# sjpark0905/DNA-LDPC-codes

Hardware: NVIDIA B200
Metric: decoded Gbit/s, n=18432 prprp (higher is better)
Workload: dtype f64

## Files before the change

dna-ldpc-codes_b200/__init__.py:

```python
import ctypes as C
import os

import numpy as np

_HERE = os.path.dirname(os.path.abspath(__file__))
LIB_PATH = os.environ.get("DNALDPC_LIB") or os.path.join(_HERE, "libdnaldpc.so")

OK = 0
PREC_F64, PREC_F32 = 0, 1
IN_LR_F64, IN_LLR_F64, IN_BSC_BITS, IN_AWGN_F32, IN_AWGN_F64, IN_VOTE_I8 = range(6)
FLAG_HOST_EXP = 1
FLAG_FIXED_ITERS = 2
FLAG_MINSUM = 4
FLAG_LAYERED = 8

EXPORTS = [
    "dnaldpc_last_error", "dnaldpc_version", "dnaldpc_code_read_pchk", "dnaldpc_code_from_csr",
    "dnaldpc_code_write_pchk", "dnaldpc_code_free", "dnaldpc_code_dims", "dnaldpc_code_export",
    "dnaldpc_code_check_regular", "dnaldpc_decoder_create", "dnaldpc_decoder_destroy", "dnaldpc_decode_batch",
    "dnaldpc_decode_batch_device", "dnaldpc_run_bp_decoder", "dnaldpc_std_dev", "dnaldpc_vote_table",
    "dnaldpc_bsc_table", "dnaldpc_synth_bsc_device", "dnaldpc_get_stats", "dnaldpc_set_profiling",
    "dnaldpc_selftest_math", "dnaldpc_redecode_sweep", "dnaldpc_get_trace", "dnaldpc_decode_window",
    "dnaldpc_redecode_sweep_ex", "dnaldpc_synth_awgn_device", "dnaldpc_synth_vote_device", "dnaldpc_code_systematic",
    "dnaldpc_encode_device", "dnaldpc_encode", "dnaldpc_extract_device", "dnaldpc_extract", "dnaldpc_simulate",
# ... 7 lines not shown


class Input(C.Structure):
    _fields_ = [("kind", C.c_int32), ("flags", C.c_int32), ("data", C.c_void_p), ("frame_stride", C.c_size_t),
                ("param", C.c_double), ("table", C.c_void_p)]


class Output(C.Structure):
    _fields_ = [("bits", C.c_void_p), ("dblk", C.c_void_p), ("iters", C.c_void_p), ("is_codeword", C.c_void_p),
                ("posterior", C.c_void_p), ("pchk", C.c_void_p)]


class Stats(C.Structure):
    _fields_ = [("frames", C.c_int64), ("frame_iters", C.c_int64), ("kernel_launches", C.c_int64),
                ("waves", C.c_int64), ("row_ms", C.c_double), ("col_ms", C.c_double), ("total_ms", C.c_double),
                ("compactions", C.c_int64)]


class Window(C.Structure):
    _fields_ = [("code_type", C.c_int32), ("L", C.c_int32), ("w", C.c_int32), ("win", C.c_int32),
                ("Mv", C.c_void_p), ("Mc", C.c_void_p)]


class Sim(C.Structure):
    _fields_ = [("channel", C.c_int32), ("flags", C.c_int32), ("param", C.c_double), ("mean_reads", C.c_double),
                ("seed", C.c_uint64), ("max_iter", C.c_int32), ("max_frames", C.c_int64), ("target_frame_errors", C.c_int64)]


class SimResult(C.Structure):
    _fields_ = [(k, C.c_int64) for k in ("frames", "iterations", "frame_errors", "bit_errors", "msg_frame_errors",
                                         "msg_bit_errors", "detected", "undetected", "raw_frame_errors", "raw_bit_errors")]
# ... 350 lines not shown
```

dna-ldpc-codes_b200/csrc/bp_kernels.cuh:

```cuda
#pragma once
#include <cuda_runtime.h>
#include <stdint.h>

#include "bp_math.cuh"
#include "rng.cuh"

namespace dnaldpc {

constexpr int kFG = 32;

template <typename T> __device__ __forceinline__ T ld_stream(const T *p) { return __ldcs(p); }
template <typename T> __device__ __forceinline__ void st_stream(T *p, T v) { __stcs(p, v); }


template <typename T>
__device__ __noinline__ void row_slow_path(T *base, const T *lr_lane, const int32_t *cols, int deg, bool fresh) {
    auto pr_at = [&](int k) -> T { return fresh ? lr_lane[(size_t)cols[k] * kFG] : base[(size_t)k * kFG]; };
    T B = T(1);
    for (int k = deg - 1; k >= 0; k--) {
        T F = T(1);
        for (int m = 0; m < k; m++) F = mul_rn(F, check_factor_slow(pr_at(m)));
        const T dk = check_factor_slow(pr_at(k));
        base[(size_t)k * kFG] = check_to_bit_slow(mul_rn(F, B));
        B = mul_rn(B, dk);
// ... 323 lines not shown
    for (int i = 0; i < 8; i++) d[i] = __hiloint2double((int)w[2 * i + 1], (int)w[2 * i]);
    ck = __hiloint2double((int)w[17], (int)w[16]);
}

__device__ __forceinline__ int nth_set_bit8(uint32_t m, int r) {
    int f = 0;
#pragma unroll
    for (int q = 0; q < 8; q++) {
        if (q == r && m) f = __ffs(m) - 1;
        m &= m - 1;
    }
    return f;
}

constexpr int kTmWarps = 12;

template <int DC, int UR>
__global__ void __launch_bounds__(kTmWarps * 32, 1)
row_pass_tmem_kernel(double *__restrict__ msg, const double *__restrict__ lratio, const uint32_t *__restrict__ actw,
                     const uint32_t *__restrict__ freshw, const int32_t *__restrict__ col_idx, int M, int N, int E,
                     int g0, int G, unsigned int *__restrict__ job_counter, int l2_hint) {
    static_assert(DC % 8 == 0 && (DC / 8) * kTmBlockCols * (kTmWarps / 4) <= 512, "tensor-memory columns");
    constexpr uint32_t kTileBytes = DC * kFG * sizeof(double);
    constexpr int NB = DC / 8, NT = DC / 4, NI = (DC + 31) / 32;
    extern __shared__ __align__(128) unsigned char smem_raw[];
    const int lane = threadIdx.x & 31, warp = threadIdx.x >> 5;
    double *tile = reinterpret_cast<double *>(smem_raw) + (size_t)warp * DC * kFG;
    unsigned char *aux = smem_raw + (size_t)kTmWarps * DC * kFG * sizeof(double);
    uint64_t *bar = reinterpret_cast<uint64_t *>(aux) + warp;
    int *sidx = reinterpret_cast<int *>(aux + kTmWarps * sizeof(uint64_t)) + warp * DC;
    uint32_t *tm_slot = reinterpret_cast<uint32_t *>(aux + kTmWarps * sizeof(uint64_t) + (size_t)kTmWarps * DC * sizeof(int));
    const double *col = tile + lane;
    const uint64_t policy = l2_evict_first_policy();
    if (warp == 0) tmem_alloc_512(tm_slot);
    if (lane == 0) {
        mbar_init(bar, 1);
        mbar_fence_init();
    }
    asm volatile("tcgen05.fence::before_thread_sync;" ::: "memory");
    __syncthreads();
    asm volatile("tcgen05.fence::after_thread_sync;" ::: "memory");
    const uint32_t tm_base = *tm_slot;
    const uint32_t taddr = tm_base + ((uint32_t)((warp & 3) * 32) << 16) + (uint32_t)((warp >> 2) * NB * kTmBlockCols);
    const unsigned njobs = (unsigned)M * (unsigned)G;
    const int kq = lane >> 3, rk = lane & 7;
    uint32_t phase = 0;

    auto start_item = [&](int g, int e0, uint32_t act, uint32_t fw, double (&v)[NT]) {
        const uint32_t fresh_mask = fw & act;
        if ((act & ~fresh_mask) != 0 && lane == 0) {
            asm volatile("fence.proxy.async.shared::cta;" ::: "memory");
            mbar_expect_tx(bar, kTileBytes);
            if (l2_hint) tma_load_1d_hint(tile, msg + ((size_t)g * E + e0) * kFG, kTileBytes, bar, policy);
            else tma_load_1d(tile, msg + ((size_t)g * E + e0) * kFG, kTileBytes, bar);
        }
        if (fresh_mask != 0) {
            const bool mine = rk < __popc(fresh_mask);
            const int f = nth_set_bit8(fresh_mask, rk);
            const double *lr_base = lratio + (size_t)g * N * kFG;
#pragma unroll
            for (int t = 0; t < NT; t++) v[t] = mine ? lr_base[(size_t)sidx[t * 4 + kq] * kFG + f] : 0.0;
        }
    };
    auto claim_raw = [&]() -> unsigned {
        unsigned j = 0;
        if (lane == 0) j = atomicAdd(job_counter, 1u);
        return j;
    };

    unsigned job = __shfl_sync(0xffffffffu, claim_raw(), 0);
    unsigned job_n = __shfl_sync(0xffffffffu, claim_raw(), 0);
    int g = 0, e0 = 0;
    uint32_t act = 0, fw = 0;
    double v[NT];
    if (job < njobs) {
        g = g0 + (int)(job / (unsigned)M);
        e0 = (int)(job % (unsigned)M) * DC;
        for (int k = lane; k < DC; k += 32) sidx[k] = __ldg(col_idx + e0 + k);
        __syncwarp();
        act = actw[g]; fw = freshw[g];
        if (act != 0) start_item(g, e0, act, fw, v);
    }
    while (job < njobs) {
        const unsigned raw_nn = claim_raw();
        const bool valid_n = job_n < njobs;
        const int g_n = g0 + (int)(job_n / (unsigned)M), e0_n = (int)(job_n % (unsigned)M) * DC;
        uint32_t act_n = 0, fw_n = 0;
        int idx_n[NI];
#pragma unroll
        for (int q = 0; q < NI; q++) idx_n[q] = 0;
        if (valid_n) {
            act_n = actw[g_n]; fw_n = freshw[g_n];
#pragma unroll
            for (int q = 0; q < NI; q++)
                if (lane + 32 * q < DC) idx_n[q] = __ldg(col_idx + e0_n + lane + 32 * q);
        }
        const bool on = (act >> lane) & 1u, fresh = (fw >> lane) & 1u;
        double *base = msg + ((size_t)g * E + e0) * kFG + lane;
        const double *lr_lane = lratio + (size_t)g * N * kFG + lane;
        const int32_t *cols_cur = col_idx + e0;
        bool bad = false;
        if (act != 0) {
            const uint32_t fresh_mask = fw & act;
            if ((act & ~fresh_mask) != 0) {
                mbar_wait(bar, phase);
                phase ^= 1u;
            }
            if (fresh_mask != 0) {
                const int nf = __popc(fresh_mask);
                {
                    const bool mine = rk < nf;
                    const int f = nth_set_bit8(fresh_mask, rk);
#pragma unroll
                    for (int t = 0; t < NT; t++)
                        if (mine) tile[(t * 4 + kq) * kFG + f] = v[t];
                }
                for (int r0 = 8; r0 < nf; r0 += 8) {
                    const int r = r0 + rk;
                    const bool mine = r < nf;
                    const int f = mine ? (int)__fns(fresh_mask, 0, r + 1) : 0;
                    double w[NT];
#pragma unroll
// ... 10 lines not shown
                double d8[8];
                const double ckb = B;
#pragma unroll
                for (int kk = 7; kk >= 0; kk--) {
                    const double dk = check_factor(col[(b * 8 + kk) * kFG], bad);
                    d8[kk] = dk;
                    B = mul_rn(B, dk);
                }
                tmem_st_block(taddr + (uint32_t)(b * kTmBlockCols), d8, ckb);
            }
            asm volatile("tcgen05.wait::st.sync.aligned;" ::: "memory");
        }
        __syncwarp();
#pragma unroll
        for (int q = 0; q < NI; q++)
            if (lane + 32 * q < DC) sidx[lane + 32 * q] = idx_n[q];
        __syncwarp();
        if (valid_n && act_n != 0) start_item(g_n, e0_n, act_n, fw_n, v);
        if (on && bad) row_slow_path<double>(base, lr_lane, cols_cur, DC, fresh);
        if (act != 0) {
            double F = 1.0;
            const bool store = on && !bad;
#pragma unroll(UR)
            for (int b = 0; b < NB; b++) {
                double d8[8], Bv[8];
                tmem_ld_block(taddr + (uint32_t)(b * kTmBlockCols), d8, Bv[7]);
#pragma unroll
                for (int kk = 7; kk > 0; kk--) Bv[kk - 1] = mul_rn(Bv[kk], d8[kk]);
#pragma unroll
                for (int kk = 0; kk < 8; kk++) {
                    const double t = mul_rn(F, Bv[kk]);
                    const double lr = check_to_bit(t);
                    if (store) st_stream(base + (size_t)(b * 8 + kk) * kFG, lr);
                    F = mul_rn(F, d8[kk]);
                }
            }
        }
        job = job_n; g = g_n; e0 = e0_n; act = act_n; fw = fw_n;
        asm volatile("shfl.sync.idx.b32 %0, %1, 0, 31, 0xffffffff;" : "=r"(job_n) : "r"(raw_nn));
    }
    asm volatile("tcgen05.fence::before_thread_sync;" ::: "memory");
    __syncthreads();
    if (warp == 0) tmem_dealloc_512(tm_base);
}

constexpr int kColWarps = 8;

template <typename T, int DV>
struct ColIn {
    int eid[DV];
    T lr[DV];
    T P;
    int deg;
};

// ... 165 lines not shown
    }
}

constexpr int kSynThreads = 256;
constexpr int kSynSplit = 64;

struct SynArgs {
    int32_t *iters_out;
    uint8_t *ok_out;
    int M, N, g0, max_iter, consider_new, fixed_iters;
    unsigned int *counter;
    unsigned int *finished;
    unsigned int *counters_to_zero;
    int clear_fresh;
    unsigned int *row_jobs;
};

constexpr int kCounterWords = 4;

__device__ __forceinline__ uint32_t syn_head(const SchedArrays &s, const SynArgs &a, int g, uint32_t &act) {
    if (a.counters_to_zero && blockIdx.x == 0 && blockIdx.y == 0 && threadIdx.x == 0) {
        a.counters_to_zero[0] = 0; a.counters_to_zero[1] = 0; a.counters_to_zero[2] = 0; a.counters_to_zero[3] = 0xffffffffu;
    }
    if (a.row_jobs && blockIdx.x == 0 && blockIdx.y == 0 && threadIdx.x == 0) *a.row_jobs = 0;
    act = s.actw[g];
    const uint32_t consider = a.consider_new ? s.newfw[g] : act;
    if (consider == 0 && a.counter && blockIdx.x == 0 && threadIdx.x == 0) {
        const unsigned add = (unsigned)(__popc(act) + __popc(s.donew[g]));
        if (add) atomicAdd(a.counter, add);
    }
    return consider;
}

template <int THREADS>
__device__ __forceinline__ void syn_tail(const SchedArrays &s, const SynArgs &a, int g, uint32_t act, uint32_t consider, uint32_t acc) {
    acc = __reduce_or_sync(0xffffffffu, acc);
    __shared__ uint32_t s_or[THREADS / 32];
    __shared__ unsigned int s_ticket;
    if ((threadIdx.x & 31) == 0) s_or[threadIdx.x >> 5] = acc;
// ... 501 lines not shown
```

dna-ldpc-codes_b200/csrc/capi.cu:

```cuda
#include <cuda_runtime.h>

#include <cmath>
#include <cstring>
#include <memory>
#include <string>
#include <thread>
#include <vector>

#include "../../include/dnaldpc.h"
#include "../host/code.h"
#include "../host/layers.h"
#include "../host/systematic.h"
#include "encoder.h"
#include "engine.h"
#include "sim.h"
#include "sources.h"

using namespace dnaldpc;

struct dnaldpc_code {
    Code c;
};
struct dnaldpc_decoder {
    Code c;
// ... 286 lines not shown
        o2.pchk = out->pchk ? t_pchk.data() : nullptr;
        rc = dnaldpc_decode_batch(d, &in2, (int64_t)K, max_iter, &o2);
        if (rc) return rc;
        for (size_t k = 0; k < K; k++) {
            const size_t f = (size_t)failed[k];
            if (out->bits) memcpy(out->bits + f * wpf, &t_bits[k * wpf], wpf * 4);
            if (out->dblk) memcpy(out->dblk + f * N, &t_dblk[k * (size_t)N], (size_t)N);
            if (out->iters) out->iters[f] = t_it[k];
            if (out->posterior) memcpy(out->posterior + f * N, &t_post[k * (size_t)N], (size_t)N * 8);
            if (out->pchk) memcpy(out->pchk + f * M, &t_pchk[k * (size_t)M], (size_t)M);
            ok[f] = t_ok[k];
            if (rounds) rounds[f] = r;
        }
        total.frames += d->stats.frames; total.frame_iters += d->stats.frame_iters;
        total.kernel_launches += d->stats.kernel_launches; total.waves += d->stats.waves;
        total.compactions += d->stats.compactions;
    }
    if (out->is_codeword) memcpy(out->is_codeword, ok.data(), (size_t)F);
    d->stats = total;
    return DNALDPC_OK;
}

int dnaldpc_redecode_sweep_ex(dnaldpc_decoder *d, const dnaldpc_input *in, int64_t F, int max_iter, const double *params,
                              int n_params, const dnaldpc_output *out, int32_t *rounds) {
    DeviceRestore restore_device;
    if (!d || !in || !out || !params || n_params <= 0 || F < 0 || max_iter < 0) return set_err(DNALDPC_ERR_ARG, "bad argument");
    if (F > 0 && !in->data) return set_err(DNALDPC_ERR_ARG, "null input buffer");
    if (in->kind == DNALDPC_IN_LR_F64) return set_err(DNALDPC_ERR_ARG, "a sweep needs a parameter to vary: LR_F64 inputs have none");
    if (in->kind == DNALDPC_IN_VOTE_I8 && in->table) return set_err(DNALDPC_ERR_ARG, "a vote-count sweep builds its tables from params[]: table must be NULL");
    for (int r = 0; r < n_params; r++) {
        dnaldpc_input t = *in;
// ... 203 lines not shown
```

dna-ldpc-codes_b200/csrc/engine.cu:

```cuda
#include "engine.h"

#include <algorithm>
#include <cmath>
#include <cstdio>
#include <cstdlib>
#include <cstring>
#include <thread>

#include "../host/layers.h"
#include "bp_kernels.cuh"
#include "layered_kernels.cuh"
#include "sw_kernels.cuh"

namespace dnaldpc {

#define CK(call)                                      \
    do {                                              \
        cudaError_t e_ = (call);                      \
        if (e_ != cudaSuccess) return fail(e_, #call); \
    } while (0)

int Engine::fail(cudaError_t e, const char *what) {
    err_ = std::string("CUDA error: ") + cudaGetErrorString(e) + " in " + what;
    return DNALDPC_ERR_CUDA;
// ... 75 lines not shown
    if (own_stream_) cudaStreamDestroy(own_stream_);
    for (auto &s : io_stream_) if (s) cudaStreamDestroy(s);
}

int Engine::ensure_slots(int G, bool want_post) {
    if (G > cap_groups_) {
        void *ptrs[] = {d_msg_, d_lratio_, d_post_, d_decw_, d_masks_, d_arrive_, d_slot_, d_mv_};
        for (void *p : ptrs) if (p) cudaFree(p);
        d_msg_ = d_lratio_ = d_post_ = nullptr; d_decw_ = d_masks_ = nullptr; d_arrive_ = nullptr; d_slot_ = d_mv_ = nullptr;
        cap_groups_ = 0;
        const size_t msg_elems = std::max<size_t>((size_t)E_, (size_t)M_ * layer_w_);
        CK(cudaMalloc(&d_msg_, std::max<size_t>((size_t)G * msg_elems * kFG * esz_, 16)));
        CK(cudaMalloc(&d_lratio_, (size_t)G * N_ * kFG * esz_));
        CK(cudaMalloc((void **)&d_decw_, (size_t)G * N_ * sizeof(uint32_t)));
        CK(cudaMalloc((void **)&d_masks_, (size_t)G * 6 * sizeof(uint32_t)));
        CK(cudaMalloc((void **)&d_arrive_, (size_t)G * sizeof(unsigned)));
        CK(cudaMalloc((void **)&d_slot_, (size_t)G * kFG * 4 * sizeof(int32_t)));
        CK(cudaMalloc((void **)&d_mv_, ((size_t)G * kFG * 2 + 2) * sizeof(int32_t)));
        cap_groups_ = G;
    }
    if (want_post && !d_post_) CK(cudaMalloc(&d_post_, (size_t)cap_groups_ * N_ * kFG * esz_));
    return DNALDPC_OK;
}

int Engine::ensure_frame_scratch(int64_t F) {
    if (F > cap_frames_) {
        if (d_iters_) cudaFree(d_iters_);
        if (d_ok_) cudaFree(d_ok_);
        d_iters_ = nullptr; d_ok_ = nullptr; cap_frames_ = 0;
        CK(cudaMalloc((void **)&d_iters_, (size_t)F * sizeof(int32_t)));
        CK(cudaMalloc((void **)&d_ok_, (size_t)F));
// ... 4 lines not shown

void Engine::fill_sched(SchedArrays &s) const {
    const size_t G = (size_t)cap_groups_;
    s.actw = d_masks_; s.donew = d_masks_ + G; s.newfw = d_masks_ + 2 * G; s.freshw = d_masks_ + 3 * G;
    s.harvw = d_masks_ + 4 * G; s.unsatw = d_masks_ + 5 * G;
    s.arrive = d_arrive_;
    const size_t S = G * kFG;
    s.slot_frame = d_slot_; s.slot_iter = d_slot_ + S; s.harv_frame = d_slot_ + 2 * S; s.harv_iter = d_slot_ + 3 * S;
    s.next_frame = d_next_;
    s.avail = d_next_ + 1;
    s.iter_sum = d_next_ + 2;
    s.in_row = d_rows_;
    s.out_row = d_rows_ + cap_rows_;
}


template <typename T> int Engine::launch_row(int g0, int G, cudaStream_t st) {
    T *msg = (T *)d_msg_;
    const T *lr = (const T *)d_lratio_;
    SchedArrays s;
    fill_sched(s);
    const long long items = (long long)G * M_;
    const unsigned grid = (unsigned)((items + kRowWarps - 1) / kRowWarps);
#define ROW(DC, EX)                                                                                                                       \
    do {                                                                                                                                  \
        if (minsum_) row_pass_kernel<T, DC, EX, ALG_MINSUM><<<grid, kRowWarps * 32, 0, st>>>(msg, lr, s.actw, s.freshw, d_row_ptr_, d_col_idx_, M_, N_, E_, g0, G); \
        else row_pass_kernel<T, DC, EX, ALG_BP><<<grid, kRowWarps * 32, 0, st>>>(msg, lr, s.actw, s.freshw, d_row_ptr_, d_col_idx_, M_, N_, E_, g0, G);         \
    } while (0)
    static const bool no_smem = getenv("DNALDPC_ROW_REGS") != nullptr;
    static const bool steady_only = getenv("DNALDPC_ROW_SMEM_STEADY_ONLY") != nullptr;
    const bool use_smem = !no_smem && (steady_ || !steady_only) && !minsum_ && sizeof(T) == 8;
    static const bool use_tmem = getenv("DNALDPC_ROW_NO_TMEM") == nullptr;
    static const int tm_hint = getenv("DNALDPC_ROW_L2HINT") ? atoi(getenv("DNALDPC_ROW_L2HINT")) : 1;
    if (use_smem && use_tmem && reg_rows_ && max_row_deg_ == 72) {
        const size_t smem = (size_t)kTmWarps * 72 * kFG * sizeof(double) + kTmWarps * sizeof(uint64_t) + (size_t)kTmWarps * 72 * sizeof(int) + 16;
        static const int ur_env = getenv("DNALDPC_ROW_UNROLL") ? atoi(getenv("DNALDPC_ROW_UNROLL")) : 0;
        const int ur = ur_env ? ur_env : (steady_ ? 9 : 3);
        if (!tmem_attr_set_) {
            CK(cudaFuncSetAttribute(row_pass_tmem_kernel<72, 1>, cudaFuncAttributeMaxDynamicSharedMemorySize, (int)smem));
            CK(cudaFuncSetAttribute(row_pass_tmem_kernel<72, 3>, cudaFuncAttributeMaxDynamicSharedMemorySize, (int)smem));
            CK(cudaFuncSetAttribute(row_pass_tmem_kernel<72, 9>, cudaFuncAttributeMaxDynamicSharedMemorySize, (int)smem));
            tmem_attr_set_ = true;
        }
        const unsigned pgrid = (unsigned)std::min<long long>((long long)sm_count_, (items + kTmWarps - 1) / kTmWarps);
        unsigned *jobs = d_counters_ + (size_t)kRing * kCounterWords;
#define TMROW(U) row_pass_tmem_kernel<72, U><<<pgrid, kTmWarps * 32, smem, st>>>((double *)msg, (const double *)lr, s.actw, s.freshw, d_col_idx_, M_, N_, E_, g0, G, jobs, tm_hint)
        if (ur == 9) TMROW(9);
        else if (ur == 3) TMROW(3);
        else TMROW(1);
#undef TMROW
    } else if (use_smem && reg_rows_ && max_row_deg_ == 72) {
        const size_t smem = (size_t)kRowWarps * 72 * kFG * sizeof(T) + kRowWarps * sizeof(uint64_t);
        bool &attr_set = smem_attr_set_[sizeof(T) == 4];
        if (!attr_set) {
            CK(cudaFuncSetAttribute(row_pass_smem_kernel<T, 72>, cudaFuncAttributeMaxDynamicSharedMemorySize, (int)smem));
            attr_set = true;
        }
        row_pass_smem_kernel<T, 72><<<grid, kRowWarps * 32, smem, st>>>(msg, lr, s.actw, s.freshw, d_row_ptr_, d_col_idx_, M_, N_, E_, g0, G);
    } else if (use_smem && max_row_deg_ <= 32 && max_row_deg_ > 8) {
        const size_t smem = (size_t)kRowWarps * 32 * kFG * sizeof(T) + kRowWarps * sizeof(uint64_t);
        row_pass_smem_kernel<T, 32, false><<<grid, kRowWarps * 32, smem, st>>>(msg, lr, s.actw, s.freshw, d_row_ptr_, d_col_idx_, M_, N_, E_, g0, G);
    } else if (reg_rows_ && max_row_deg_ == 72) ROW(72, true);
    else if (max_row_deg_ <= 8) ROW(8, false);
    else if (max_row_deg_ <= 32) ROW(32, false);
    else if (max_row_deg_ <= 72) ROW(72, false);
// ... 57 lines not shown
        stats.kernel_launches++;
    }
    CK(cudaGetLastError());
    return DNALDPC_OK;
}

int Engine::launch_syndrome(const dnaldpc_output &out, int G, int max_iter, int consider_new, int fixed, unsigned *counter,
                            unsigned *finished, unsigned *rearm, int clear_fresh, cudaStream_t st) {
    SchedArrays s;
    fill_sched(s);
    SynArgs a;
    a.iters_out = out.iters; a.ok_out = out.is_codeword;
    a.M = M_; a.N = N_; a.g0 = 0; a.max_iter = max_iter; a.consider_new = consider_new; a.fixed_iters = fixed;
    a.counter = counter; a.finished = finished; a.counters_to_zero = rearm; a.clear_fresh = clear_fresh;
    a.row_jobs = d_counters_ + (size_t)kRing * kCounterWords;
    const size_t smem = (size_t)N_ * sizeof(uint32_t);
    static const bool no_smem = getenv("DNALDPC_SYN_GATHER") != nullptr;
    if (!no_smem && smem <= (size_t)kSynSmemGate && N_ % 4 == 0) {
        if (!syn_attr_set_) {
            CK(cudaFuncSetAttribute(syndrome_update_smem_kernel, cudaFuncAttributeMaxDynamicSharedMemorySize, kSynSmemGate));
            syn_attr_set_ = true;
        }
        static const int split = getenv("DNALDPC_SYN_SPLIT") ? std::max(1, atoi(getenv("DNALDPC_SYN_SPLIT"))) : kSynSmemSplit;
        syndrome_update_smem_kernel<<<dim3((unsigned)split, (unsigned)G), kSynSmemThreads, smem, st>>>(d_decw_, s, a, d_row_ptr_, d_col_idx_);
    } else if (!no_smem && (size_t)N_ * sizeof(uint16_t) <= (size_t)kSynHalfGate && N_ % 4 == 0) {
        if (!syn_half_attr_set_) {
            CK(cudaFuncSetAttribute(syndrome_update_half_kernel, cudaFuncAttributeMaxDynamicSharedMemorySize, kSynHalfGate));
            syn_half_attr_set_ = true;
        }
        syndrome_update_half_kernel<<<dim3(kSynSmemSplit, (unsigned)G, 2), kSynSmemThreads, (size_t)N_ * sizeof(uint16_t), st>>>(d_decw_, s, a, d_row_ptr_, d_col_idx_);
// ... 194 lines not shown
                const int msg_elems = layered_ ? M_ * layer_w_ : E_;
                dim3 mgrid((unsigned)((msg_elems + N_ + kMoveThreads * kMoveUnroll - 1) / (kMoveThreads * kMoveUnroll)),
                           (unsigned)std::min<unsigned>(std::max(last_inuse, 1u), 2048u));
                compact_move_kernel<T><<<mgrid, kMoveThreads, 0, st>>>((T *)d_msg_, (T *)d_lratio_, mv_src, mv_dst, mv_cnt, N_, msg_elems);
                stats.kernel_launches += 2;
                stats.compactions++;
                CK(cudaGetLastError());
                G_rc = (int)std::min<long long>(G, ((long long)last_inuse + kFG - 1) / kFG);
                G_rc = std::max(G_rc, 1);
                packed_cap = (long long)G_rc * kFG;
            }
        }
        const bool trace = trace_ticks_ > 0 && tick >= 8 && tick < 8 + kTrace && tick < 8 + trace_ticks_;
        if (trace) CK(cudaEventRecord(trace_ev_[3 * (tick - 8)], st));
        if (profiling) CK(cudaEventRecord(prof_ev_[0], st));
        rc = layered_ ? launch_layers<T>(G_rc, st) : launch_row<T>(0, G_rc, st);
        if (rc) return rc;
        if (profiling) CK(cudaEventRecord(prof_ev_[1], st));
        if (trace) CK(cudaEventRecord(trace_ev_[3 * (tick - 8) + 1], st));
        if (!layered_) rc = launch_col<T>(0, G_rc, want_post, st);
        if (rc) return rc;
        if (trace) { CK(cudaEventRecord(trace_ev_[3 * (tick - 8) + 2], st)); traced_ = (int)(tick - 8) + 1; }
        if (profiling) {
            CK(cudaEventRecord(prof_ev_[2], st));
            CK(cudaEventSynchronize(prof_ev_[2]));
            float a_ms = 0, b_ms = 0;
            cudaEventElapsedTime(&a_ms, prof_ev_[0], prof_ev_[1]);
            cudaEventElapsedTime(&b_ms, prof_ev_[1], prof_ev_[2]);
            stats.row_ms += a_ms;
            stats.col_ms += b_ms;
            stats.waves++;
        }
    }
    unsigned long long it_sum = 0;
    CK(cudaMemcpyAsync(&it_sum, d_next_ + 2, sizeof(it_sum), cudaMemcpyDeviceToHost, st));
// ... 498 lines not shown
```

dna-ldpc-codes_b200/csrc/engine.h:

```cpp
#pragma once
#include <cuda_runtime.h>

#include <atomic>
#include <cstdint>
#include <string>
#include <vector>

#include "../../include/dnaldpc.h"
#include "../host/code.h"

namespace dnaldpc {

struct SchedArrays;
class Engine;

struct Session {
    dnaldpc_input in;
    dnaldpc_output out;
    int max_iter = 0;
    int64_t max_frames = 0;
};

class FrameSource {
  public:
// ... 28 lines not shown
                   double read_err, int8_t *out_k, cudaStream_t stream, uint64_t cw_off = 0);

    dnaldpc_stats stats{};
    bool profiling = false;
    double minsum_scale = 1.0;
    int trace_ticks_ = 0;
    int trace_result(double *row_ms, double *col_ms, double *sched_ms);

  private:
    template <typename T> int run(const Session &ss, FrameSource &src, cudaStream_t st);
    int sw_groups(const Code &code, const dnaldpc_window &w, const std::vector<int> &sched, const double *lratio, int64_t F,
                  int max_iter, const dnaldpc_output &out, int G);
    int sw_lockstep(const dnaldpc_window &w, const std::vector<int> &sched, const double *lratio, int64_t F, int max_iter,
                    const dnaldpc_output &out, int G);
    int ensure_rows(int64_t frames);
    template <typename T> int launch_row(int g0, int G, cudaStream_t st);
    template <typename T> int launch_col(int g0, int G, bool want_post, cudaStream_t st);
    template <typename T> int launch_layers(int G, cudaStream_t st);
    template <typename T> int launch_harvest_setup(const dnaldpc_input &in, const dnaldpc_output &out, int g0, int G, cudaStream_t st);
    int launch_syndrome(const dnaldpc_output &out, int G, int max_iter, int consider_new, int fixed, unsigned *counter,
                        unsigned *finished, unsigned *rearm, int clear_fresh, cudaStream_t st);
    int ensure_slots(int groups, bool want_post);
    int ensure_frame_scratch(int64_t F);
    int fail(cudaError_t e, const char *what);
    int fail(const std::string &m, int rc);
    void fill_sched(SchedArrays &s) const;

    std::string err_;
    int device_ = 0, precision_ = 0, wave_frames_ = 4096, sm_count_ = 148;
    int M_ = 0, N_ = 0, E_ = 0, max_row_deg_ = 0, max_col_deg_ = 0;
    bool reg_rows_ = false, reg_cols_ = false;
// ... 76 lines not shown
```

dna-ldpc-codes_b200/csrc/sim.cu:

```cuda
#include "sim.h"

#include <algorithm>
#include <atomic>
#include <chrono>
#include <cstdlib>
#include <deque>
#include <map>
#include <mutex>
#include <thread>

#include "rng.cuh"

namespace dnaldpc {

namespace {

enum { kIters, kFrameErr, kBitErr, kMsgFrameErr, kMsgBitErr, kDetected, kUndetected, kRawFrameErr, kRawBitErr, kCounters };
enum { kRecBits, kRecMsgBits, kRecRawBits, kRecIters, kRecFlags, kRecWords };
enum { kFlagFrameErr = 1, kFlagMsgFrameErr = 2, kFlagDetected = 4, kFlagUndetected = 8, kFlagRawFrameErr = 16 };
constexpr int kCountWarps = 8;

__global__ void __launch_bounds__(256)
sim_message_kernel(uint64_t seed, long long f0, int n, int kw, int K, uint32_t *__restrict__ msg) {
    const long long t = (long long)blockIdx.x * blockDim.x + threadIdx.x;
// ... 67 lines not shown
#pragma unroll
        for (int k = 0; k < kCounters; k++) part[warp][k] = v[k];
    __syncthreads();
    if (threadIdx.x < kCounters) {
        unsigned long long s = 0;
#pragma unroll
        for (int w = 0; w < kCountWarps; w++) s += part[w][threadIdx.x];
        if (s) atomicAdd(cnt + threadIdx.x, s);
    }
}

int64_t round_up(int64_t x, int64_t m) { return (x + m - 1) / m * m; }

void add_stats(dnaldpc_stats &a, const dnaldpc_stats &s) {
    a.frames += s.frames; a.frame_iters += s.frame_iters; a.kernel_launches += s.kernel_launches; a.waves += s.waves;
    a.row_ms += s.row_ms; a.col_ms += s.col_ms; a.compactions += s.compactions;
}

struct PieceResult {
    int64_t n = 0;
    int64_t cnt[kCounters] = {};
    std::vector<int32_t> rec;
};

struct SimShared {
    int64_t F = 0, T = 0, P = 0, n_pieces = 0;
    std::atomic<int64_t> next_piece{0};
    std::atomic<bool> stop{false};
    std::mutex mu;
    std::map<int64_t, PieceResult> pending;
    int64_t folded = 0;
// ... 317 lines not shown
```

dna-ldpc-codes_b200/csrc/sources.cu:

```cuda
#include "sources.h"

#include <algorithm>
#include <atomic>
#include <chrono>
#include <cmath>
#include <condition_variable>
#include <cstdio>
#include <cstdlib>
#include <cstring>
#include <mutex>
#include <thread>

namespace dnaldpc {

size_t packed_stride(int kind, int N) {
    switch (kind) {
        case DNALDPC_IN_LR_F64: case DNALDPC_IN_LLR_F64: case DNALDPC_IN_AWGN_F64: return (size_t)N * 8;
        case DNALDPC_IN_AWGN_F32: return (size_t)N * 4;
        case DNALDPC_IN_BSC_BITS: return (size_t)((N + 31) / 32) * 4;
        case DNALDPC_IN_VOTE_I8: return (size_t)N;
    }
    return 0;
}

static void add_stats(dnaldpc_stats &a, const dnaldpc_stats &s) {
    a.frames += s.frames; a.frame_iters += s.frame_iters; a.kernel_launches += s.kernel_launches; a.waves += s.waves;
    a.row_ms += s.row_ms; a.col_ms += s.col_ms; a.compactions += s.compactions;
}

static int64_t round_up(int64_t x, int64_t m) { return (x + m - 1) / m * m; }


namespace {

struct HostBatch {
    dnaldpc_input in;
    dnaldpc_output out;
    int64_t F = 0;
    int max_iter = 0, N = 0, M = 0, chunk = 32, exp_threads = 1;
    size_t stride = 0, packed = 0, wpf = 0;
    int64_t n_chunks = 0;
    std::atomic<int64_t> next_chunk{0};
// ... 606 lines not shown
```

include/dnaldpc.h:

```cpp
#ifndef DNALDPC_H
#define DNALDPC_H
#include <stddef.h>
#include <stdint.h>

#ifdef __cplusplus
extern "C" {
#endif

#define DNALDPC_OK 0
#define DNALDPC_ERR_ARG 1
#define DNALDPC_ERR_IO 2
#define DNALDPC_ERR_FORMAT 3
#define DNALDPC_ERR_CUDA 4
#define DNALDPC_ERR_NOMEM 5
#define DNALDPC_ERR_UNSUPPORTED 6

typedef struct dnaldpc_code dnaldpc_code;
typedef struct dnaldpc_decoder dnaldpc_decoder;

const char *dnaldpc_last_error(void);
const char *dnaldpc_version(void);


int dnaldpc_code_read_pchk(const char *path, dnaldpc_code **out);
// ... 104 lines not shown
    int64_t frame_errors, bit_errors;
    int64_t msg_frame_errors, msg_bit_errors;
    int64_t detected, undetected;
    int64_t raw_frame_errors, raw_bit_errors;
} dnaldpc_sim_result;
int dnaldpc_simulate(dnaldpc_decoder *d, const dnaldpc_sim *s, dnaldpc_sim_result *r);

typedef struct dnaldpc_stats {
    int64_t frames;
    int64_t frame_iters;
    int64_t kernel_launches;
    int64_t waves;
    double row_ms, col_ms;
    double total_ms;
    int64_t compactions;
} dnaldpc_stats;
int dnaldpc_get_stats(const dnaldpc_decoder *d, dnaldpc_stats *s);
int dnaldpc_set_profiling(dnaldpc_decoder *d, int on);
int dnaldpc_get_trace(dnaldpc_decoder *d, double *row_ms, double *col_ms, double *sched_ms, int *ticks);

int dnaldpc_selftest_math(int64_t n, uint64_t seed, int64_t *mismatches);

#ifdef __cplusplus
}
#endif
#endif
```

Measured before the change: 0.2392.

## Fuse row and column BP passes into one persistent tick kernel with group readiness flags

Merges the check-node (row) pass and the bit-node (column) pass into a single persistent TMEM kernel. Column work items for a frame group are interleaved with row items and gated on a per-group completion counter that uses release/acquire flags, so the separate column kernel launch and its global barrier go away. Bit items gather their edge messages with per-edge TMA loads (or cp.async when an environment flag is set) and write posteriors and decisions directly. This adds spin-wait dependencies and uncoalesced gathers, and it leaves temporary clock64 diagnostics and env-driven knobs in the hot loop.

Result: slower. 0.1592, median of 6 (-33.5%).

```diff
diff --git a/dna-ldpc-codes_b200/__init__.py b/dna-ldpc-codes_b200/__init__.py
--- a/dna-ldpc-codes_b200/__init__.py
+++ b/dna-ldpc-codes_b200/__init__.py
@@ -45,7 +45,7 @@
 class Stats(C.Structure):
     _fields_ = [("frames", C.c_int64), ("frame_iters", C.c_int64), ("kernel_launches", C.c_int64),
                 ("waves", C.c_int64), ("row_ms", C.c_double), ("col_ms", C.c_double), ("total_ms", C.c_double),
-                ("compactions", C.c_int64)]
+                ("compactions", C.c_int64), ("fused_ticks", C.c_int64)]
 
 
 class Window(C.Structure):
diff --git a/dna-ldpc-codes_b200/csrc/bp_kernels.cuh b/dna-ldpc-codes_b200/csrc/bp_kernels.cuh
--- a/dna-ldpc-codes_b200/csrc/bp_kernels.cuh
+++ b/dna-ldpc-codes_b200/csrc/bp_kernels.cuh
@@ -361,22 +361,47 @@
 }
 
 constexpr int kTmWarps = 12;
-
-template <int DC, int UR>
+constexpr int kFusedBits = 9;
+
+struct TickArgs {
+    double *msg;
+    const double *lratio;
+    const uint32_t *actw, *freshw;
+    const int32_t *col_idx, *col_edge;
+    uint32_t *decw;
+    double *post;
+    unsigned int *job_counter;
+    unsigned int *grp_done;
+    int M, N, E, g0, G;
+    int head;
+    int l2_hint;
+    int tmp_gather;
+    unsigned long long *tmp_diag;
+};
+
+__device__ __forceinline__ unsigned ld_acquire_gpu(const unsigned *p) {
+    unsigned v;
+    asm volatile("ld.acquire.gpu.global.u32 %0, [%1];" : "=r"(v) : "l"(p) : "memory");
+    return v;
+}
+
+template <int DC, int UR, bool FUSED>
 __global__ void __launch_bounds__(kTmWarps * 32, 1)
-row_pass_tmem_kernel(double *__restrict__ msg, const double *__restrict__ lratio, const uint32_t *__restrict__ actw,
-                     const uint32_t *__restrict__ freshw, const int32_t *__restrict__ col_idx, int M, int N, int E,
-                     int g0, int G, unsigned int *__restrict__ job_counter, int l2_hint) {
+tick_fused_kernel(TickArgs a) {
     static_assert(DC % 8 == 0 && (DC / 8) * kTmBlockCols * (kTmWarps / 4) <= 512, "tensor-memory columns");
+    static_assert(!FUSED || DC == 8 * kFusedBits, "a bit item fills one check item's tile");
     constexpr uint32_t kTileBytes = DC * kFG * sizeof(double);
     constexpr int NB = DC / 8, NT = DC / 4, NI = (DC + 31) / 32;
+    double *__restrict__ msg = a.msg;
+    const double *__restrict__ lratio = a.lratio;
+    const int M = a.M, N = a.N, E = a.E, g0 = a.g0;
     extern __shared__ __align__(128) unsigned char smem_raw[];
     const int lane = threadIdx.x & 31, warp = threadIdx.x >> 5;
     double *tile = reinterpret_cast<double *>(smem_raw) + (size_t)warp * DC * kFG;
     unsigned char *aux = smem_raw + (size_t)kTmWarps * DC * kFG * sizeof(double);
     uint64_t *bar = reinterpret_cast<uint64_t *>(aux) + warp;
-    int *sidx = reinterpret_cast<int *>(aux + kTmWarps * sizeof(uint64_t)) + warp * DC;
-    uint32_t *tm_slot = reinterpret_cast<uint32_t *>(aux + kTmWarps * sizeof(uint64_t) + (size_t)kTmWarps * DC * sizeof(int));
+    int *sidx2 = reinterpret_cast<int *>(aux + kTmWarps * sizeof(uint64_t)) + warp * 2 * DC;
+    uint32_t *tm_slot = reinterpret_cast<uint32_t *>(aux + kTmWarps * sizeof(uint64_t) + (size_t)kTmWarps * 2 * DC * sizeof(int));
     const double *col = tile + lane;
     const uint64_t policy = l2_evict_first_policy();
     if (warp == 0) tmem_alloc_512(tm_slot);
@@ -389,16 +414,72 @@
     asm volatile("tcgen05.fence::after_thread_sync;" ::: "memory");
     const uint32_t tm_base = *tm_slot;
     const uint32_t taddr = tm_base + ((uint32_t)((warp & 3) * 32) << 16) + (uint32_t)((warp >> 2) * NB * kTmBlockCols);
-    const unsigned njobs = (unsigned)M * (unsigned)G;
+    const unsigned gm = (unsigned)M * (unsigned)a.G;
+    const unsigned njobs = FUSED ? 2u * gm : gm;
+    const unsigned head = FUSED ? min((unsigned)a.head, gm) : gm;
     const int kq = lane >> 3, rk = lane & 7;
     uint32_t phase = 0;
 
-    auto start_item = [&](int g, int e0, uint32_t act, uint32_t fw, double (&v)[NT]) {
+    auto decode = [&](unsigned p, bool &bit, int &g, int &e0) {
+        unsigned x = p;
+        bit = false;
+        if (FUSED && p >= head) {
+            const unsigned t = p - head, alt = 2u * (gm - head);
+            if (t >= alt) { bit = true; x = gm - head + (t - alt); }
+            else if (t & 1u) x = head + (t >> 1);
+            else { bit = true; x = t >> 1; }
+        }
+        g = g0 + (int)(x / (unsigned)M);
+        e0 = (int)(x % (unsigned)M) * DC;
+    };
+    auto group_ready = [&](int g, bool block) -> bool {
+        unsigned ok = 0;
+        if (lane == 0) {
+            unsigned d = ld_acquire_gpu(a.grp_done + g);
+            while (block && d < (unsigned)M) {
+                __nanosleep(128);
+                d = ld_acquire_gpu(a.grp_done + g);
+            }
+            ok = d >= (unsigned)M;
+            if (ok) asm volatile("fence.proxy.async.global;" ::: "memory");
+        }
+        return __shfl_sync(0xffffffffu, ok, 0) != 0;
+    };
+    auto start_item = [&](bool bit, int g, int e0, uint32_t act, uint32_t fw, const int *sx, double (&v)[NT]) {
+        if (FUSED && bit && a.tmp_gather) {
+            __syncwarp();
+            const double *gmsg = msg + (size_t)g * E * kFG;
+#pragma unroll 6
+            for (int t = 0; t < DC / 2; t++) {
+                const int c = lane + 32 * t, k = c >> 4, off = (c & 15) * 2;
+                asm volatile("cp.async.cg.shared.global.L2::cache_hint [%0], [%1], 16, %2;" ::"r"(smem_u32(tile + k * kFG + off)),
+                             "l"(gmsg + (size_t)sx[k] * kFG + off), "l"(policy) : "memory");
+            }
+            asm volatile("cp.async.commit_group;" ::: "memory");
+            const double *lr_lane = lratio + ((size_t)g * N + e0 / 8) * kFG + lane;
+#pragma unroll
+            for (int b = 0; b < kFusedBits; b++) v[b] = __ldg(lr_lane + (size_t)b * kFG);
+            return;
+        }
+        if (FUSED && bit) {
+            if (lane == 0) {
+                asm volatile("fence.proxy.async.shared::cta;" ::: "memory");
+                mbar_expect_tx(bar, kTileBytes);
+                const double *gmsg = msg + (size_t)g * E * kFG;
+#pragma unroll 8
+                for (int k = 0; k < DC; k++)
+                    tma_load_1d_hint(tile + k * kFG, gmsg + (size_t)sx[k] * kFG, kFG * sizeof(double), bar, policy);
+            }
+            const double *lr_lane = lratio + ((size_t)g * N + e0 / 8) * kFG + lane;
+#pragma unroll
+            for (int b = 0; b < kFusedBits; b++) v[b] = __ldg(lr_lane + (size_t)b * kFG);
+            return;
+        }
         const uint32_t fresh_mask = fw & act;
         if ((act & ~fresh_mask) != 0 && lane == 0) {
             asm volatile("fence.proxy.async.shared::cta;" ::: "memory");
             mbar_expect_tx(bar, kTileBytes);
-            if (l2_hint) tma_load_1d_hint(tile, msg + ((size_t)g * E + e0) * kFG, kTileBytes, bar, policy);
+            if (a.l2_hint) tma_load_1d_hint(tile, msg + ((size_t)g * E + e0) * kFG, kTileBytes, bar, policy);
             else tma_load_1d(tile, msg + ((size_t)g * E + e0) * kFG, kTileBytes, bar);
         }
         if (fresh_mask != 0) {
@@ -406,53 +487,84 @@
             const int f = nth_set_bit8(fresh_mask, rk);
             const double *lr_base = lratio + (size_t)g * N * kFG;
 #pragma unroll
-            for (int t = 0; t < NT; t++) v[t] = mine ? lr_base[(size_t)sidx[t * 4 + kq] * kFG + f] : 0.0;
+            for (int t = 0; t < NT; t++) v[t] = mine ? lr_base[(size_t)sx[t * 4 + kq] * kFG + f] : 0.0;
         }
     };
     auto claim_raw = [&]() -> unsigned {
         unsigned j = 0;
-        if (lane == 0) j = atomicAdd(job_counter, 1u);
+        if (lane == 0) j = atomicAdd(a.job_counter, 1u);
         return j;
     };
 
+    long long dg[10] = {0, 0, 0, 0, 0, 0, 0, 0, 0, 0};
+    const long long tk0 = clock64();
     unsigned job = __shfl_sync(0xffffffffu, claim_raw(), 0);
     unsigned job_n = __shfl_sync(0xffffffffu, claim_raw(), 0);
-    int g = 0, e0 = 0;
+    bool bit = false, started = false;
+    int g = 0, e0 = 0, buf = 0;
     uint32_t act = 0, fw = 0;
     double v[NT];
     if (job < njobs) {
-        g = g0 + (int)(job / (unsigned)M);
-        e0 = (int)(job % (unsigned)M) * DC;
-        for (int k = lane; k < DC; k += 32) sidx[k] = __ldg(col_idx + e0 + k);
+        decode(job, bit, g, e0);
+        const int32_t *tab = (FUSED && bit) ? a.col_edge : a.col_idx;
+        for (int k = lane; k < DC; k += 32) sidx2[k] = __ldg(tab + e0 + k);
         __syncwarp();
-        act = actw[g]; fw = freshw[g];
-        if (act != 0) start_item(g, e0, act, fw, v);
+        act = a.actw[g]; fw = a.freshw[g];
     }
     while (job < njobs) {
+        int *sidx = sidx2 + buf * DC, *sidx_n = sidx2 + (buf ^ 1) * DC;
+        long long tq0 = clock64();
+        if (!started && act != 0) {
+            dg[0] += 1;
+            if (FUSED && bit) group_ready(g, true);
+            start_item(bit, g, e0, act, fw, sidx, v);
+        }
         const unsigned raw_nn = claim_raw();
         const bool valid_n = job_n < njobs;
-        const int g_n = g0 + (int)(job_n / (unsigned)M), e0_n = (int)(job_n % (unsigned)M) * DC;
+        bool bit_n = false;
+        int g_n = 0, e0_n = 0;
+        if (valid_n) decode(job_n, bit_n, g_n, e0_n);
         uint32_t act_n = 0, fw_n = 0;
         int idx_n[NI];
 #pragma unroll
         for (int q = 0; q < NI; q++) idx_n[q] = 0;
         if (valid_n) {
-            act_n = actw[g_n]; fw_n = freshw[g_n];
+            act_n = a.actw[g_n]; fw_n = a.freshw[g_n];
+            const int32_t *tab = (FUSED && bit_n) ? a.col_edge : a.col_idx;
 #pragma unroll
             for (int q = 0; q < NI; q++)
-                if (lane + 32 * q < DC) idx_n[q] = __ldg(col_idx + e0_n + lane + 32 * q);
+                if (lane + 32 * q < DC) idx_n[q] = __ldg(tab + e0_n + lane + 32 * q);
         }
         const bool on = (act >> lane) & 1u, fresh = (fw >> lane) & 1u;
         double *base = msg + ((size_t)g * E + e0) * kFG + lane;
         const double *lr_lane = lratio + (size_t)g * N * kFG + lane;
-        const int32_t *cols_cur = col_idx + e0;
+        const int32_t *cols_cur = a.col_idx + e0;
         bool bad = false;
-        if (act != 0) {
+        long long tq1 = clock64(); dg[1] += tq1 - tq0;
+        if (act != 0 && FUSED && bit) {
+            if (a.tmp_gather) {
+                asm volatile("cp.async.wait_group 0;" ::: "memory");
+                __syncwarp();
+            } else {
+            mbar_wait(bar, phase);
+            phase ^= 1u;
+            }
+            { long long t = clock64(); dg[2] += t - tq1; dg[6] += 1; }
+#pragma unroll
+            for (int b = 0; b < kFusedBits; b++) {
+                double d8[8];
+#pragma unroll
+                for (int kk = 0; kk < 8; kk++) d8[kk] = col[(b * 8 + kk) * kFG];
+                tmem_st_block(taddr + (uint32_t)(b * kTmBlockCols), d8, v[b]);
+            }
+            asm volatile("tcgen05.wait::st.sync.aligned;" ::: "memory");
+        } else if (act != 0) {
             const uint32_t fresh_mask = fw & act;
             if ((act & ~fresh_mask) != 0) {
                 mbar_wait(bar, phase);
                 phase ^= 1u;
             }
+            { long long t = clock64(); dg[3] += t - tq1; dg[7] += 1; }
             if (fresh_mask != 0) {
                 const int nf = __popc(fresh_mask);
                 {
@@ -493,31 +605,84 @@
         __syncwarp();
 #pragma unroll
         for (int q = 0; q < NI; q++)
-            if (lane + 32 * q < DC) sidx[lane + 32 * q] = idx_n[q];
+            if (lane + 32 * q < DC) sidx_n[lane + 32 * q] = idx_n[q];
         __syncwarp();
-        if (valid_n && act_n != 0) start_item(g_n, e0_n, act_n, fw_n, v);
-        if (on && bad) row_slow_path<double>(base, lr_lane, cols_cur, DC, fresh);
-        if (act != 0) {
-            double F = 1.0;
-            const bool store = on && !bad;
+        bool started_n = false;
+        if (valid_n && act_n != 0 && (!(FUSED && bit_n) || group_ready(g_n, false))) {
+            start_item(bit_n, g_n, e0_n, act_n, fw_n, sidx_n, v);
+            started_n = true;
+        }
+        if (FUSED && bit) {
+            if (act != 0) {
+                double *gmsg = msg + (size_t)g * E * kFG + lane;
+                const int j0 = e0 / 8;
 #pragma unroll(UR)
-            for (int b = 0; b < NB; b++) {
-                double d8[8], Bv[8];
-                tmem_ld_block(taddr + (uint32_t)(b * kTmBlockCols), d8, Bv[7]);
-#pragma unroll
-                for (int kk = 7; kk > 0; kk--) Bv[kk - 1] = mul_rn(Bv[kk], d8[kk]);
-#pragma unroll
-                for (int kk = 0; kk < 8; kk++) {
-                    const double t = mul_rn(F, Bv[kk]);
-                    const double lr = check_to_bit(t);
-                    if (store) st_stream(base + (size_t)(b * 8 + kk) * kFG, lr);
-                    F = mul_rn(F, d8[kk]);
+                for (int b = 0; b < kFusedBits; b++) {
+                    double lr[8], P;
+                    tmem_ld_block(taddr + (uint32_t)(b * kTmBlockCols), lr, P);
+                    double p[8];
+#pragma unroll
+                    for (int k = 0; k < 8; k++) {
+                        p[k] = P;
+                        P = mul_rn(P, lr[k]);
+                    }
+                    if (P != P) P = 1.0;
+                    if (a.post != nullptr && on) a.post[((size_t)g * N + j0 + b) * kFG + lane] = P;
+                    double S = 1.0;
+#pragma unroll
+                    for (int k = 7; k >= 0; k--) {
+                        double w = mul_rn(p[k], S);
+                        if (w != w) w = 1.0;
+                        if (on) st_stream(gmsg + (size_t)sidx[b * 8 + k] * kFG, w);
+                        S = mul_rn(S, lr[k]);
+                    }
+                    const uint32_t wb = __ballot_sync(0xffffffffu, on ? P <= 1.0 : true);
+                    if (lane == 0) {
+                        uint32_t *dst = a.decw + (size_t)g * N + j0 + b;
+                        *dst = (act == 0xffffffffu) ? wb : ((wb & act) | (*dst & ~act));
+                    }
                 }
             }
-        }
-        job = job_n; g = g_n; e0 = e0_n; act = act_n; fw = fw_n;
+        } else {
+            if (on && bad) row_slow_path<double>(base, lr_lane, cols_cur, DC, fresh);
+            if (act != 0) {
+                double F = 1.0;
+                const bool store = on && !bad;
+#pragma unroll(UR)
+                for (int b = 0; b < NB; b++) {
+                    double d8[8], Bv[8];
+                    tmem_ld_block(taddr + (uint32_t)(b * kTmBlockCols), d8, Bv[7]);
+#pragma unroll
+                    for (int kk = 7; kk > 0; kk--) Bv[kk - 1] = mul_rn(Bv[kk], d8[kk]);
+#pragma unroll
+                    for (int kk = 0; kk < 8; kk++) {
+                        const double t = mul_rn(F, Bv[kk]);
+                        const double lr = check_to_bit(t);
+                        if (store) {
+                            if (FUSED) base[(size_t)(b * 8 + kk) * kFG] = lr;
+                            else st_stream(base + (size_t)(b * 8 + kk) * kFG, lr);
+                        }
+                        F = mul_rn(F, d8[kk]);
+                    }
+                }
+            }
+            if (FUSED) {
+                long long tf = clock64();
+                asm volatile("fence.proxy.async.global;" ::: "memory");
+                __syncwarp();
+                if (lane == 0) asm volatile("red.release.gpu.global.add.u32 [%0], 1;" ::"l"(a.grp_done + g) : "memory");
+                __syncwarp();
+                dg[4] += clock64() - tf;
+            }
+        }
+        if (FUSED && bit) dg[8] += clock64() - tq0; else dg[9] += clock64() - tq0;
+        job = job_n; bit = bit_n; g = g_n; e0 = e0_n; act = act_n; fw = fw_n; started = started_n; buf ^= 1;
         asm volatile("shfl.sync.idx.b32 %0, %1, 0, 31, 0xffffffff;" : "=r"(job_n) : "r"(raw_nn));
     }
+    dg[5] = clock64() - tk0;
+    if (a.tmp_diag && lane == 0)
+#pragma unroll
+        for (int q = 0; q < 10; q++) atomicAdd(a.tmp_diag + q, (unsigned long long)dg[q]);
     asm volatile("tcgen05.fence::before_thread_sync;" ::: "memory");
     __syncthreads();
     if (warp == 0) tmem_dealloc_512(tm_base);
@@ -713,6 +878,7 @@
     unsigned int *counters_to_zero;
     int clear_fresh;
     unsigned int *row_jobs;
+    unsigned int *grp_done;
 };
 
 constexpr int kCounterWords = 4;
@@ -722,6 +888,7 @@
         a.counters_to_zero[0] = 0; a.counters_to_zero[1] = 0; a.counters_to_zero[2] = 0; a.counters_to_zero[3] = 0xffffffffu;
     }
     if (a.row_jobs && blockIdx.x == 0 && blockIdx.y == 0 && threadIdx.x == 0) *a.row_jobs = 0;
+    if (a.grp_done && blockIdx.x == 0 && blockIdx.z == 0 && threadIdx.x == 0) a.grp_done[g] = 0;
     act = s.actw[g];
     const uint32_t consider = a.consider_new ? s.newfw[g] : act;
     if (consider == 0 && a.counter && blockIdx.x == 0 && threadIdx.x == 0) {
diff --git a/dna-ldpc-codes_b200/csrc/capi.cu b/dna-ldpc-codes_b200/csrc/capi.cu
--- a/dna-ldpc-codes_b200/csrc/capi.cu
+++ b/dna-ldpc-codes_b200/csrc/capi.cu
@@ -324,7 +324,7 @@
         }
         total.frames += d->stats.frames; total.frame_iters += d->stats.frame_iters;
         total.kernel_launches += d->stats.kernel_launches; total.waves += d->stats.waves;
-        total.compactions += d->stats.compactions;
+        total.compactions += d->stats.compactions; total.fused_ticks += d->stats.fused_ticks;
     }
     if (out->is_codeword) memcpy(out->is_codeword, ok.data(), (size_t)F);
     d->stats = total;
diff --git a/dna-ldpc-codes_b200/csrc/engine.cu b/dna-ldpc-codes_b200/csrc/engine.cu
--- a/dna-ldpc-codes_b200/csrc/engine.cu
+++ b/dna-ldpc-codes_b200/csrc/engine.cu
@@ -113,7 +113,7 @@
         CK(cudaMalloc(&d_lratio_, (size_t)G * N_ * kFG * esz_));
         CK(cudaMalloc((void **)&d_decw_, (size_t)G * N_ * sizeof(uint32_t)));
         CK(cudaMalloc((void **)&d_masks_, (size_t)G * 6 * sizeof(uint32_t)));
-        CK(cudaMalloc((void **)&d_arrive_, (size_t)G * sizeof(unsigned)));
+        CK(cudaMalloc((void **)&d_arrive_, (size_t)G * 2 * sizeof(unsigned)));
         CK(cudaMalloc((void **)&d_slot_, (size_t)G * kFG * 4 * sizeof(int32_t)));
         CK(cudaMalloc((void **)&d_mv_, ((size_t)G * kFG * 2 + 2) * sizeof(int32_t)));
         cap_groups_ = G;
@@ -148,6 +148,75 @@
     s.out_row = d_rows_ + cap_rows_;
 }
 
+
+template <typename T> bool Engine::tmem_rows() const {
+    static const bool no_smem = getenv("DNALDPC_ROW_REGS") != nullptr;
+    static const bool steady_only = getenv("DNALDPC_ROW_SMEM_STEADY_ONLY") != nullptr;
+    static const bool use_tmem = getenv("DNALDPC_ROW_NO_TMEM") == nullptr;
+    return !no_smem && (steady_ || !steady_only) && !minsum_ && sizeof(T) == 8 && use_tmem && reg_rows_ && max_row_deg_ == 72;
+}
+
+constexpr int kFusedHeadHalves = 4;
+
+int Engine::launch_tmem(int G, bool fused, bool want_post, cudaStream_t st) {
+    const size_t smem = (size_t)kTmWarps * 72 * kFG * sizeof(double) + kTmWarps * sizeof(uint64_t) + (size_t)kTmWarps * 2 * 72 * sizeof(int) + 16;
+    static const int ur_env = getenv("DNALDPC_ROW_UNROLL") ? atoi(getenv("DNALDPC_ROW_UNROLL")) : 0;
+    static const int tm_hint = getenv("DNALDPC_ROW_L2HINT") ? atoi(getenv("DNALDPC_ROW_L2HINT")) : 1;
+    const int ur = ur_env ? ur_env : (steady_ ? 9 : 3);
+    if (!tmem_attr_set_) {
+        CK(cudaFuncSetAttribute(tick_fused_kernel<72, 1, false>, cudaFuncAttributeMaxDynamicSharedMemorySize, (int)smem));
+        CK(cudaFuncSetAttribute(tick_fused_kernel<72, 3, false>, cudaFuncAttributeMaxDynamicSharedMemorySize, (int)smem));
+        CK(cudaFuncSetAttribute(tick_fused_kernel<72, 9, false>, cudaFuncAttributeMaxDynamicSharedMemorySize, (int)smem));
+        CK(cudaFuncSetAttribute(tick_fused_kernel<72, 1, true>, cudaFuncAttributeMaxDynamicSharedMemorySize, (int)smem));
+        CK(cudaFuncSetAttribute(tick_fused_kernel<72, 3, true>, cudaFuncAttributeMaxDynamicSharedMemorySize, (int)smem));
+        CK(cudaFuncSetAttribute(tick_fused_kernel<72, 9, true>, cudaFuncAttributeMaxDynamicSharedMemorySize, (int)smem));
+        tmem_attr_set_ = true;
+    }
+    SchedArrays s;
+    fill_sched(s);
+    TickArgs a;
+    a.msg = (double *)d_msg_; a.lratio = (const double *)d_lratio_; a.actw = s.actw; a.freshw = s.freshw;
+    a.col_idx = d_col_idx_; a.col_edge = d_col_edge_; a.decw = d_decw_; a.post = want_post ? (double *)d_post_ : nullptr;
+    a.job_counter = d_counters_ + (size_t)kRing * kCounterWords;
+    a.grp_done = d_arrive_ + cap_groups_;
+    a.M = M_; a.N = N_; a.E = E_; a.g0 = 0; a.G = G;
+    static const int hh_tmp = getenv("TMP_HEAD_HALVES") ? atoi(getenv("TMP_HEAD_HALVES")) : kFusedHeadHalves;
+    a.head = M_ + (hh_tmp - 2) * (M_ / 2);
+    a.l2_hint = tm_hint;
+    static const int tmp_gather = getenv("TMP_GATHER") ? atoi(getenv("TMP_GATHER")) : 0;
+    a.tmp_gather = tmp_gather;
+    static unsigned long long *tmp_diag = nullptr;
+    static int tmp_n = 0;
+    a.tmp_diag = nullptr;
+    if (getenv("TMP_DIAG") && fused) {
+        if (!tmp_diag) { cudaMalloc(&tmp_diag, 10 * 8); }
+        tmp_n++;
+        if (tmp_n == 50) { cudaMemsetAsync(tmp_diag, 0, 80, st); a.tmp_diag = tmp_diag; }
+        if (tmp_n == 51) {
+            unsigned long long h[10];
+            cudaMemcpy(h, tmp_diag, 80, cudaMemcpyDeviceToHost);
+            fprintf(stderr, "TMPDIAG G=%d ur=%d deferred=%llu defer_cyc=%llu bitwait_cyc=%llu checkwait_cyc=%llu release_cyc=%llu total_cyc=%llu bits=%llu checks=%llu bit_item_cyc=%llu check_item_cyc=%llu\n",
+                    G, ur, h[0], h[1], h[2], h[3], h[4], h[5], h[6], h[7], h[8], h[9]);
+        }
+    }
+    const long long items = (long long)G * M_ * (fused ? 2 : 1);
+    const unsigned pgrid = (unsigned)std::min<long long>((long long)sm_count_, (items + kTmWarps - 1) / kTmWarps);
+#define TM(U, F) tick_fused_kernel<72, U, F><<<pgrid, kTmWarps * 32, smem, st>>>(a)
+    if (fused) {
+        if (ur == 9) TM(9, true);
+        else if (ur == 3) TM(3, true);
+        else TM(1, true);
+        stats.fused_ticks++;
+    } else {
+        if (ur == 9) TM(9, false);
+        else if (ur == 3) TM(3, false);
+        else TM(1, false);
+    }
+#undef TM
+    stats.kernel_launches++;
+    CK(cudaGetLastError());
+    return DNALDPC_OK;
+}
 
 template <typename T> int Engine::launch_row(int g0, int G, cudaStream_t st) {
     T *msg = (T *)d_msg_;
@@ -164,25 +233,8 @@
     static const bool no_smem = getenv("DNALDPC_ROW_REGS") != nullptr;
     static const bool steady_only = getenv("DNALDPC_ROW_SMEM_STEADY_ONLY") != nullptr;
     const bool use_smem = !no_smem && (steady_ || !steady_only) && !minsum_ && sizeof(T) == 8;
-    static const bool use_tmem = getenv("DNALDPC_ROW_NO_TMEM") == nullptr;
-    static const int tm_hint = getenv("DNALDPC_ROW_L2HINT") ? atoi(getenv("DNALDPC_ROW_L2HINT")) : 1;
-    if (use_smem && use_tmem && reg_rows_ && max_row_deg_ == 72) {
-        const size_t smem = (size_t)kTmWarps * 72 * kFG * sizeof(double) + kTmWarps * sizeof(uint64_t) + (size_t)kTmWarps * 72 * sizeof(int) + 16;
-        static const int ur_env = getenv("DNALDPC_ROW_UNROLL") ? atoi(getenv("DNALDPC_ROW_UNROLL")) : 0;
-        const int ur = ur_env ? ur_env : (steady_ ? 9 : 3);
-        if (!tmem_attr_set_) {
-            CK(cudaFuncSetAttribute(row_pass_tmem_kernel<72, 1>, cudaFuncAttributeMaxDynamicSharedMemorySize, (int)smem));
-            CK(cudaFuncSetAttribute(row_pass_tmem_kernel<72, 3>, cudaFuncAttributeMaxDynamicSharedMemorySize, (int)smem));
-            CK(cudaFuncSetAttribute(row_pass_tmem_kernel<72, 9>, cudaFuncAttributeMaxDynamicSharedMemorySize, (int)smem));
-            tmem_attr_set_ = true;
-        }
-        const unsigned pgrid = (unsigned)std::min<long long>((long long)sm_count_, (items + kTmWarps - 1) / kTmWarps);
-        unsigned *jobs = d_counters_ + (size_t)kRing * kCounterWords;
-#define TMROW(U) row_pass_tmem_kernel<72, U><<<pgrid, kTmWarps * 32, smem, st>>>((double *)msg, (const double *)lr, s.actw, s.freshw, d_col_idx_, M_, N_, E_, g0, G, jobs, tm_hint)
-        if (ur == 9) TMROW(9);
-        else if (ur == 3) TMROW(3);
-        else TMROW(1);
-#undef TMROW
+    if (tmem_rows<T>()) {
+        return launch_tmem(G, false, false, st);
     } else if (use_smem && reg_rows_ && max_row_deg_ == 72) {
         const size_t smem = (size_t)kRowWarps * 72 * kFG * sizeof(T) + kRowWarps * sizeof(uint64_t);
         bool &attr_set = smem_attr_set_[sizeof(T) == 4];
@@ -270,6 +322,7 @@
     a.M = M_; a.N = N_; a.g0 = 0; a.max_iter = max_iter; a.consider_new = consider_new; a.fixed_iters = fixed;
     a.counter = counter; a.finished = finished; a.counters_to_zero = rearm; a.clear_fresh = clear_fresh;
     a.row_jobs = d_counters_ + (size_t)kRing * kCounterWords;
+    a.grp_done = d_arrive_ + cap_groups_;
     const size_t smem = (size_t)N_ * sizeof(uint32_t);
     static const bool no_smem = getenv("DNALDPC_SYN_GATHER") != nullptr;
     if (!no_smem && smem <= (size_t)kSynSmemGate && N_ % 4 == 0) {
@@ -494,11 +547,13 @@
         const bool trace = trace_ticks_ > 0 && tick >= 8 && tick < 8 + kTrace && tick < 8 + trace_ticks_;
         if (trace) CK(cudaEventRecord(trace_ev_[3 * (tick - 8)], st));
         if (profiling) CK(cudaEventRecord(prof_ev_[0], st));
-        rc = layered_ ? launch_layers<T>(G_rc, st) : launch_row<T>(0, G_rc, st);
+        const bool fused = !layered_ && !profiling && reg_cols_ && max_col_deg_ == 8 && tmem_rows<T>();
+        if (fused) rc = launch_tmem(G_rc, true, want_post, st);
+        else rc = layered_ ? launch_layers<T>(G_rc, st) : launch_row<T>(0, G_rc, st);
         if (rc) return rc;
         if (profiling) CK(cudaEventRecord(prof_ev_[1], st));
         if (trace) CK(cudaEventRecord(trace_ev_[3 * (tick - 8) + 1], st));
-        if (!layered_) rc = launch_col<T>(0, G_rc, want_post, st);
+        if (!layered_ && !fused) rc = launch_col<T>(0, G_rc, want_post, st);
         if (rc) return rc;
         if (trace) { CK(cudaEventRecord(trace_ev_[3 * (tick - 8) + 2], st)); traced_ = (int)(tick - 8) + 1; }
         if (profiling) {
diff --git a/dna-ldpc-codes_b200/csrc/engine.h b/dna-ldpc-codes_b200/csrc/engine.h
--- a/dna-ldpc-codes_b200/csrc/engine.h
+++ b/dna-ldpc-codes_b200/csrc/engine.h
@@ -66,7 +66,9 @@
     int sw_lockstep(const dnaldpc_window &w, const std::vector<int> &sched, const double *lratio, int64_t F, int max_iter,
                     const dnaldpc_output &out, int G);
     int ensure_rows(int64_t frames);
+    template <typename T> bool tmem_rows() const;
     template <typename T> int launch_row(int g0, int G, cudaStream_t st);
+    int launch_tmem(int G, bool fused, bool want_post, cudaStream_t st);
     template <typename T> int launch_col(int g0, int G, bool want_post, cudaStream_t st);
     template <typename T> int launch_layers(int G, cudaStream_t st);
     template <typename T> int launch_harvest_setup(const dnaldpc_input &in, const dnaldpc_output &out, int g0, int G, cudaStream_t st);
diff --git a/dna-ldpc-codes_b200/csrc/sim.cu b/dna-ldpc-codes_b200/csrc/sim.cu
--- a/dna-ldpc-codes_b200/csrc/sim.cu
+++ b/dna-ldpc-codes_b200/csrc/sim.cu
@@ -105,7 +105,7 @@
 
 void add_stats(dnaldpc_stats &a, const dnaldpc_stats &s) {
     a.frames += s.frames; a.frame_iters += s.frame_iters; a.kernel_launches += s.kernel_launches; a.waves += s.waves;
-    a.row_ms += s.row_ms; a.col_ms += s.col_ms; a.compactions += s.compactions;
+    a.row_ms += s.row_ms; a.col_ms += s.col_ms; a.compactions += s.compactions; a.fused_ticks += s.fused_ticks;
 }
 
 struct PieceResult {
diff --git a/dna-ldpc-codes_b200/csrc/sources.cu b/dna-ldpc-codes_b200/csrc/sources.cu
--- a/dna-ldpc-codes_b200/csrc/sources.cu
+++ b/dna-ldpc-codes_b200/csrc/sources.cu
@@ -25,7 +25,7 @@
 
 static void add_stats(dnaldpc_stats &a, const dnaldpc_stats &s) {
     a.frames += s.frames; a.frame_iters += s.frame_iters; a.kernel_launches += s.kernel_launches; a.waves += s.waves;
-    a.row_ms += s.row_ms; a.col_ms += s.col_ms; a.compactions += s.compactions;
+    a.row_ms += s.row_ms; a.col_ms += s.col_ms; a.compactions += s.compactions; a.fused_ticks += s.fused_ticks;
 }
 
 static int64_t round_up(int64_t x, int64_t m) { return (x + m - 1) / m * m; }
diff --git a/include/dnaldpc.h b/include/dnaldpc.h
--- a/include/dnaldpc.h
+++ b/include/dnaldpc.h
@@ -142,6 +142,7 @@
     double row_ms, col_ms;
     double total_ms;
     int64_t compactions;
+    int64_t fused_ticks;
 } dnaldpc_stats;
 int dnaldpc_get_stats(const dnaldpc_decoder *d, dnaldpc_stats *s);
 int dnaldpc_set_profiling(dnaldpc_decoder *d, int on);
```
